# bwiberg/beam-radiance-estimate-pbrt

Measured on AMD Instinct MI355X. Metric: beam-radiance estimates/sec at 1M photons, higher is better.
Workload: dtype fp32

## Files before the change

### beam-radiance-estimate-pbrt_amd/csrc/bre_api_check.hip

```cpp
#include <cmath>
#include <cstring>
#include <vector>

#include "bre_ctx.h"

using namespace bre;

namespace {

bre_status check_hierarchy(bre_ctx *c, int64_t n, const float *x, int32_t n_aux, const float *aux, float *y) {
    if (n_aux < 2 || !aux) return fail(c, BRE_ERR_INVALID_ARG, "bre_device_check: kind 10 needs aux = (key_lo, leaf_size)");
    const int key_lo = (int)aux[0], K = (int)aux[1];
    if (n < 8 || n % 8 || !x || !y || key_lo < 0 || key_lo > 63 || K < 1 || K > 64 || n / 8 > ((int64_t)1 << 24))
        return fail(c, BRE_ERR_INVALID_ARG, "bre_device_check: kind 10 needs m <= 2^24 keys and boxes (8 words each), "
                    "key_lo in 0..63 and leaf_size in 1..64");
    const int64_t m = n / 8;
    std::vector<unsigned long long> keys((size_t)m);
    std::memcpy(keys.data(), x, (size_t)m * 8);
    for (int64_t i = 1; i < m; ++i)
        if ((keys[(size_t)i] >> key_lo) < (keys[(size_t)i - 1] >> key_lo))
            return fail(c, BRE_ERR_INVALID_ARG, "bre_device_check: kind 10 keys >> %d decrease at %lld: the hierarchy "
                        "kernels need a non-decreasing sequence", key_lo, (long long)i);
    std::vector<BeamRec> recs((size_t)m);
    const float *bx = x + 2 * m;
// ... 55 lines not shown
    int32_t head[8] = {0, 0, K, c->built_key_lo, (int32_t)nn, has4 ? 1 : 0, (int32_t)nleaf, 0};
    std::memcpy(head, &nv, sizeof(int64_t));
    std::memcpy(y, head, sizeof(head));
    if (nv == 0) return BRE_OK;
    BRE_TRY(set_device(c));
    float *keys = y + 8, *idx = keys + 2 * nv, *box = idx + nv, *nodes = box + 6 * nv, *lp = nodes + 16 * nn,
          *nodes4 = lp + nleaf;
    std::vector<BeamRec> recs((size_t)nv);
    HIPCHK(c, hipMemcpyAsync(keys, c->sort.keys_alt.ptr, (size_t)nv * 8, hipMemcpyDeviceToHost, c->stream));
    HIPCHK(c, hipMemcpyAsync(idx, c->sort.vals_alt.ptr, (size_t)nv * 4, hipMemcpyDeviceToHost, c->stream));
    HIPCHK(c, hipMemcpyAsync(recs.data(), c->recs.ptr, (size_t)nv * sizeof(BeamRec), hipMemcpyDeviceToHost, c->stream));
    HIPCHK(c, hipMemcpyAsync(nodes, c->nodes.ptr, (size_t)nn * sizeof(Node), hipMemcpyDeviceToHost, c->stream));
    if (nleaf > 1)
        HIPCHK(c, hipMemcpyAsync(lp, c->leaf_parent.ptr, (size_t)nleaf * 4, hipMemcpyDeviceToHost, c->stream));
    if (has4)
        HIPCHK(c, hipMemcpyAsync(nodes4, c->nodes4.ptr, (size_t)nn * sizeof(Node4), hipMemcpyDeviceToHost, c->stream));
    HIPCHK(c, hipStreamSynchronize(c->stream));
    if (nleaf == 1) std::memset(lp, 0, 4);
    for (int64_t i = 0; i < nv; ++i)
        for (int k = 0; k < 3; ++k) {
            box[6 * i + k] = recs[(size_t)i].lo[k];
            box[6 * i + 3 + k] = recs[(size_t)i].hi[k];
        }
    return BRE_OK;
}

}

extern "C" {

bre_status bre_device_check(bre_ctx *c, int32_t kind, int64_t n, const float *x, int32_t n_aux, const float *aux,
                            float *y) {
    if (!c) return BRE_ERR_INVALID_ARG;
    if (kind < 0 || kind > 14) return fail(c, BRE_ERR_INVALID_ARG, "bre_device_check: kind %d not in [0, 14]", kind);
    if (kind == 10) return check_hierarchy(c, n, x, n_aux, aux, y);
    if (kind == 11) return check_read_tree(c, n, y);
    if (n < 0 || (n > 0 && (!x || !y))) return fail(c, BRE_ERR_INVALID_ARG, "bre_device_check: bad arrays");
    if (kind == 12) {
        if (n % 6) return fail(c, BRE_ERR_INVALID_ARG, "bre_device_check: kind 12 needs whole records of 6 floats");
        if (n == 0) return BRE_OK;
        BRE_TRY(set_device(c));
        float *dx = nullptr, *dy = nullptr;
        HIPCHK(c, c->chk_x.get((size_t)n, &dx));
        HIPCHK(c, c->chk_y.get((size_t)n, &dy));
        HIPCHK(c, hipMemcpyAsync(dx, x, (size_t)n * 4, hipMemcpyHostToDevice, c->stream));
        HIPCHK(c, launch_check_specular(n / 6, dx, dy, c->stream));
        HIPCHK(c, hipMemcpyAsync(y, dy, (size_t)n * 4, hipMemcpyDeviceToHost, c->stream));
        HIPCHK(c, hipStreamSynchronize(c->stream));
        return BRE_OK;
    }
    if (kind == 13) {
        constexpr int kWords = (int)(sizeof(bre_material_ex) / 4);
        if (n % 9 || n_aux < kWords || n_aux % kWords || !aux)
            return fail(c, BRE_ERR_INVALID_ARG, "bre_device_check: kind 13 needs whole records of 9 floats and, in aux, "
                        "whole bre_material_ex records of %d words", kWords);
        const int n_mats = n_aux / kWords;
        std::vector<bre_material_ex> mats((size_t)n_mats);
        std::memcpy(mats.data(), aux, (size_t)n_aux * 4);
        std::vector<DevBsdf> table((size_t)n_mats);
        for (int k = 0; k < n_mats; ++k) {
            const std::string what = check_glossy_material(mats[(size_t)k]);
            if (!what.empty())
                return fail(c, BRE_ERR_INVALID_ARG, "bre_device_check: kind 13: material %d has %s", k, what.c_str());
            table[(size_t)k] = make_bsdf(mats[(size_t)k]);
        }
        for (int64_t i = 0; i < n / 9; ++i)
            if (!(x[9 * i + 8] >= 0 && x[9 * i + 8] < (float)n_mats) || x[9 * i + 8] != std::floor(x[9 * i + 8]))
                return fail(c, BRE_ERR_INVALID_ARG, "bre_device_check: kind 13: record %lld names material %g of %d",
                            (long long)i, (double)x[9 * i + 8], n_mats);
        if (n == 0) return BRE_OK;
// ... 167 lines not shown
```

### beam-radiance-estimate-pbrt_amd/csrc/bre_api_gather.hip

```cpp
#include <algorithm>

#include "bre_ctx.h"

using namespace bre;

namespace {

bre_status read_counters(bre_ctx *c, DevCounters *ctr) {
    if (!(c->timing || c->counters)) return BRE_OK;
    DevCounters h;
    HIPCHK(c, hipMemcpyAsync(&h, ctr, sizeof(h), hipMemcpyDeviceToHost, c->stream));
    HIPCHK(c, hipStreamSynchronize(c->stream));
    if (c->timing) {
        float ms = 0.f;
        HIPCHK(c, hipEventElapsedTime(&ms, c->ev[2], c->ev[3]));
        c->stats.gather_ms = ms;
    }
    c->stats.candidates = (int64_t)h.candidates;
    c->stats.contributions = (int64_t)h.contributions;
    c->stats.node_visits = (int64_t)h.node_visits;
    c->stats.leaf_visits = (int64_t)h.leaf_visits;
    c->stats.beam_evals = (int64_t)h.beam_evals;
    c->stats.ccp_wave_evals = (int64_t)h.ccp_wave_evals;
    c->stats.prefilter_rejects = (int64_t)h.prefilter_rejects;
// ... 121 lines not shown
    a.prefilter = c->prefilter;
    a.occupancy = c->occupancy;
    a.block_map = c->block_map;
    a.tscan = c->tscan >= 0 ? c->tscan : tscan_for(R + c->bset.radius);
    a.margin = c->margin;
    a.stack_cap = c->stack_cap;
    a.tile_spec = c->tile_spec;
    a.tile_budget = c->tile_budget;
    c->stats.tile_variant = 0;
    a.tile_variant = &c->stats.tile_variant;
    c->stats.n_segments = nseg;
    if (c->nvalid == 0) {
        HIPCHK(c, launch_zero_outputs(a, c->stream));
        return BRE_OK;
    }
    const int kernel = c->kernel;
    if (c->shard_mode == 2 && c->shard_count > 1 && (kernel == 2 || kernel == 5))
        return fail(c, BRE_ERR_STATE, "work-root shards (BRE_OPT_SHARD_MODE 2) need the tile kernel (BRE_OPT_KERNEL 0 or 4)");
    if (kernel == 5) {
        if (seg_index) return fail(c, BRE_ERR_STATE, "kernel 5 gathers in the caller's order only");
        return gather_chunk(c, a);
    }
    if (kernel == 2 && seg_index) return fail(c, BRE_ERR_STATE, "kernel 2 gathers in the caller's order only");
    if (kernel == 2) {
        if (c->timing) HIPCHK(c, hipEventRecord(c->ev[2], c->stream));
        HIPCHK(c, launch_gather_thread(a, c->counters, c->stream));
        if (c->timing) HIPCHK(c, hipEventRecord(c->ev[3], c->stream));
        return read_counters(c, a.ctr);
    }
    const bool want_cnt = c->counters || out.seg_counts;
    const bool rshard = c->shard_mode == 2 && c->shard_count > 1;
    const int S_eff = rshard ? (c->split + c->shard_count - 1) / c->shard_count : c->split;
    const size_t per_seg = (size_t)S_eff * (12 + (want_cnt ? 8 : 0));
    int64_t chunk = c->partial_cap / (int64_t)per_seg / 64 * 64;
    if (chunk > ((int64_t)1 << 26)) chunk = (int64_t)1 << 26;
    if (chunk < 64) chunk = 64;
    if (chunk > nseg) chunk = nseg;
    int32_t *roots = nullptr;
    HIPCHK(c, c->roots.get(kMaxSplit + 1, &roots));
    HIPCHK(c, c->partial.get(3 * (size_t)chunk * (size_t)S_eff, &a.partial));
    if (c->roots_split != c->split) {
        HIPCHK(c, c->roots_tmp.ensure(roots_scratch_bytes()));
        HIPCHK(c, launch_roots(a.nodes, c->split, roots, c->roots_tmp.ptr, c->stream));
        c->roots_split = c->split;
    }
    if (!c->nodes4_ok) {
        Node4 *nodes4 = nullptr;
        HIPCHK(c, c->nodes4.get((size_t)c->nnodes, &nodes4));
        HIPCHK(c, launch_collapse4(a.nodes, c->nnodes, nodes4, c->stream));
        c->nodes4_ok = true;
    }
    a.nodes4 = c->nodes4.as<Node4>();
    a.roots = roots;
    if (rshard) {
        int32_t *roots_sh = nullptr;
        HIPCHK(c, c->roots_sh.get(kMaxSplit + 1, &roots_sh));
        HIPCHK(c, launch_roots_shard(roots, c->split, c->shard_rank, c->shard_count, S_eff, roots_sh, c->stream));
        a.roots = roots_sh;
        a.split = S_eff;
    }
    HIPCHK(c, c->segrec.get((size_t)((chunk + 63) / 64 * 64), &a.segrec));
    if (want_cnt) HIPCHK(c, c->pcnt.get(2 * (size_t)chunk * (size_t)S_eff, &a.pcnt));
    if (c->tile_axis && a.leaf_size > 0) {
        const int64_t ntiles = (c->nvalid + a.leaf_size - 1) / a.leaf_size;
        HIPCHK(c, c->tileax.get((size_t)ntiles, &a.tileax));
        HIPCHK(c, c->segbox.get(8, &a.segbox));
    }
    if (c->timing) HIPCHK(c, hipEventRecord(c->ev[2], c->stream));
    if (!c->tile_ev) HIPCHK(c, hipEventCreateWithFlags(&c->tile_ev.h, hipEventDisableTiming));
    for (int64_t off = 0; off < nseg; off += chunk) {
        GatherArgs ac = a;
        ac.wait_ev = (off == 0 && c->after && c->after->tile_ev_valid) ? c->after->tile_ev.h : nullptr;
        ac.done_ev = off + chunk >= nseg ? c->tile_ev.h : nullptr;
        ac.user_start = off == 0 ? c->user_ev[0] : nullptr;
        ac.user_end = off + chunk >= nseg ? c->user_ev[1] : nullptr;
        ac.nseg = std::min(chunk, nseg - off);
        ac.seg = seg.slice(off);
        if (seg_index)
            ac.seg_index = seg_index + off;
        else
            ac.out = out.slice(off);
        HIPCHK(c, launch_gather_tile(ac, c->counters, c->stream));
    }
    c->tile_ev_valid = true;
    if (c->timing) HIPCHK(c, hipEventRecord(c->ev[3], c->stream));
    return read_counters(c, a.ctr);
}

bre_status gather_segments_core(bre_ctx *c, int64_t n, const SegView &seg, float R, int64_t npix,
                                const GatherOut &out) {
    const bool pshard = c->shard_mode == 1 && c->shard_count > 1;
    const bool sortable = c->kernel == 0 || c->kernel == 4;
    const bool seg_out = out.seg_rgb || out.seg_counts;
    if (n < 0 || npix < 0) return fail(c, BRE_ERR_INVALID_ARG, "bre_gather: negative size");
    if (n > 0 && (!seg.o || !seg.p || !seg.d || !seg.t))
        return fail(c, BRE_ERR_INVALID_ARG, "bre_gather: null segment array");
    if (out.accum && !seg.pix) return fail(c, BRE_ERR_INVALID_ARG, "bre_gather: accum_rgb given without seg_pixel");
    if (pshard && seg_out) {
        if (!sortable) return fail(c, BRE_ERR_STATE, "packet shards with per-segment outputs need kernel 0 or 4");
        GatherArgs z{};
        z.nseg = n;
        z.out = out;
        HIPCHK(c, launch_zero_outputs(z, c->stream));
    }
    const auto pick = [&](const SegView &from, const int32_t *index) -> bre_status {
        const int64_t m = bre_shard_segments(n, c->shard_rank, c->shard_count, c->shard_block);
        c->stats.n_segments = m;
        if (m == 0) return BRE_OK;
        SegArrays &sp = c->sp;
        int32_t *sp_index = nullptr;
        HIPCHK(c, sp.ensure((size_t)m));
        if (seg_out) HIPCHK(c, c->sp_index.get((size_t)m, &sp_index));
        const PacketPick pk{n, m, c->shard_rank, c->shard_count, c->shard_block, from, index, sp.out(), sp_index};
        HIPCHK(c, launch_packet_pick(pk, c->stream));
        SegView picked = sp.view();
// ... 185 lines not shown
```

### beam-radiance-estimate-pbrt_amd/csrc/bre_ctx.h

```cpp
#pragma once
#include <hip/hip_runtime.h>

#include <cstddef>
#include <cstdint>
#include <cstring>
#include <initializer_list>
#include <string>
#include <vector>

#include "../../include/bre.h"
#include "bre_device.h"
#include "bre_trace.h"

#ifndef BRE_KERNEL_READBACK
#define BRE_KERNEL_READBACK 1
#endif
#ifndef BRE_TILE_BUDGET
#define BRE_TILE_BUDGET 7
#endif
static_assert(BRE_TILE_BUDGET == 6 || BRE_TILE_BUDGET == 7, "BRE_TILE_BUDGET must be 6 or 7");

namespace bre {

struct NoCopy {
// ... 143 lines not shown
};

struct SceneDevice {
    DevMem tris, nodes, prims, light_tri, light_func, light_cdf, dlights, mats, bsdfs, lobes, lobes_mx;
    DevScene head;
    uint64_t hash = 0;
    std::vector<unsigned char> bytes[4];
    DevMem md_table, md_pairs, md_light, md_dens;
    bool media_stale = false;
    DevMem grid;
    std::vector<unsigned char> grid_bytes;
    DevMem record;
    std::vector<unsigned char> record_bytes;
};

}

struct bre_ctx {
    int device = 0;
    bre::Stream stream;
    bre::Stream pstream;
    bre::Event ev[4];
    bre::Event fork_ev, join_ev;
    bre::Event tile_ev;
    bool tile_ev_valid = false;
    hipEvent_t user_ev[2] = {nullptr, nullptr};
    bre::PinnedWords flags_host;
    bre::PinnedWords rb_host;
    std::string err;
    bool counters = false, timing = false, prefilter = true, sort_segments = true;
    int kernel = 0, leaf_size = 1, sqrt_mode = 0, split = 256, leaf2 = 64, chunk_len = 400, chunk_leaf = 1;
    int shard_rank = 0, shard_count = 1, shard_block = 1, shard_mode = 0, film_classes = 1;
    int stack_cap = 0, occupancy = 6, sort_key = 4, block_map = 3, tscan = -1;
    int64_t partial_cap = (int64_t)4 << 30;
    int beam_key = 2, margin = 1, tile_axis = 1, split_records = 0, film_compose = 1;
    int photon_single = 1, pass_priority = 1, kernel_readback = BRE_KERNEL_READBACK;
    int slot_passes = 1, coarse_keys = 0, stage_all = 0, tile_spec = 1;
    int tile_budget = BRE_TILE_BUDGET;
    int64_t nbeams = 0, nvalid = 0, nnodes = 0;
    bre::BeamSet bset;
    int built_leaf_size = 1;
    int built_key_lo = 0;
    bool build_scratch_ok = false;
    int roots_split = -1;
    bool nodes4_ok = false;
    bool beams_kept = false;
    bre::BeamArrays in;
    bre::DevMem box, cent, cbounds, nvalid_buf, leaf_parent, visit, gbox;
    bre::SortScratch sort;
    bre::DevMem recs, pow, nodes;
    bre::SegArrays g;
    bre::DevMem g_accum, g_seg_rgb, g_counts;
    bre::DevMem counters_buf, roots, roots_sh, roots_tmp, partial, pcnt, segrec, tileax, segbox, nodes4;
    bre::DevMem ch_bounds, ch_counts, ch_offsets, ch_range, ch_scan_tmp, ch_box, ch_cent, ch_slo, ch_shi, ch_par,
        ch_recs, ch_cpar, ch_nodes;
    int64_t n_chunks = 0;
    bre::DevMem ss_bounds;
    bre::SortScratch ss_sort;
    bre::SegArrays ss;
    bre::SegArrays sp;
    bre::DevMem sp_index;
    bre::DevMem px_seg, px_cls;
    bre::SortScratch px_sort;
    bre::SceneState held;
    bre::SceneDevice dev;
    int seg_budget = 16;
    bre::DevMem ph_counts, ph_offsets, ph_tmp;
    bre::BeamArrays ph_s;
    bre::DevMem cam_dev, cam_perms, cam_offs, cam_tmp, cam_flags;
    bre::SegArrays cs;
    bre::DevMem cs_valid;
    bre::SegArrays seg;
    bre::DevMem seg_depth;
    int64_t cam_nseg = 0;
    int64_t cam_npix = 0;
    int cam_w = -1, cam_h = -1;
    bre_scene cam_scene;
    bre::DevMem chk_x, chk_aux, chk_y;
    int lds_per_block = 0;
    bre_stats stats;
    bre_ctx *after = nullptr;
    std::vector<bre_ctx *> followers;
};

namespace bre {

// ... 81 lines not shown
```

### beam-radiance-estimate-pbrt_amd/csrc/bre_device.h

```cpp
#pragma once

#include <hip/hip_runtime.h>
#include <stdint.h>

#include "bre_views.h"

namespace bre {

struct alignas(16) BeamRec {
    float lo[3], hi[3];
    float b0[3];
    float bu[3];
    float mag_b;
    float radius;
    float pad[2];
};
struct BeamSet {
    int uniform = 0;
    float radius = 0.f;
};
__device__ __forceinline__ float beam_radius(const BeamSet &u, float rec_radius) {
    return u.uniform ? u.radius : rec_radius;
}
static_assert(sizeof(BeamRec) == 64, "BeamRec must be one 64-B line");

struct alignas(16) Node {
    float lo[2][3];
    float hi[2][3];
    int32_t child[2];
    int32_t parent;
    int32_t nleaf;
};
static_assert(sizeof(Node) == 64, "Node must be one 64-B line");

constexpr int32_t kEmptyChild = INT32_MIN;

struct alignas(16) Node4 {
// ... 77 lines not shown
    float invs[3];
    float inv_mag_a;
};
static_assert(sizeof(SegRec) == 64, "SegRec must be one 64-B line");
__device__ __forceinline__ const float4 *seg_plane(const SegRec *base, int64_t s, int k) {
    return reinterpret_cast<const float4 *>(base) + ((s >> 6) << 8) + (k << 6) + (s & 63);
}

struct alignas(16) TileAxis {
    float d[3], thr;
    float m[3], grow;
};

struct GatherArgs {
    int64_t nseg;
    SegView seg;
    float R;
    int64_t npix;
    GatherOut out;
    const int32_t *seg_index;
    const BeamRec *recs;
    const float4 *pow;
    BeamSet bset;
    const Node *nodes;
    const Node4 *nodes4 = nullptr;
    int64_t nvalid;
    int leaf_size;
    DevCounters *ctr;
    const int32_t *roots;
    int split;
    float *partial;
    int32_t *pcnt;
    SegRec *segrec;
    bool prefilter;
    int occupancy;
    int stack_cap;
    int block_map;
    int tscan;
    int margin;
    int tile_spec = 1;
    int tile_budget = 7;
    int64_t *tile_variant = nullptr;
    TileAxis *tileax;
    unsigned int *segbox;
    hipEvent_t wait_ev = nullptr;
    hipEvent_t done_ev = nullptr;
    hipEvent_t user_start = nullptr, user_end = nullptr;
};

struct ChunkBuild {
    const BeamRec *parents;
    BeamSet bset;
    int64_t nparents;
    const float *seg_o, *seg_p;
    int64_t nseg;
    float R;
    float len_factor;
    unsigned int *seg_bounds;
    unsigned int *cbounds;
    int32_t *counts;
    int64_t *offsets;
    float *range;
    void *scan_tmp;
    size_t scan_tmp_bytes;
};
size_t chunk_scan_temp_bytes(int64_t n);
// ... 44 lines not shown
    const uint8_t *cls;
    int classes;
    unsigned int *keys, *keys_alt;
    int32_t *vals, *vals_alt;
    void *tmp;
    size_t tmp_bytes;
    unsigned int *flags;
    unsigned int bad_pixel_flag;
    int slot = 1;
};
size_t pixel_sort_temp_bytes(int64_t n);
hipError_t launch_pixel_compose(const PixelCompose &c, hipStream_t st);
hipError_t launch_seg_classes(int64_t n, int block, int classes, const int32_t *perm, uint8_t *cls, hipStream_t st);
hipError_t launch_film_add(int64_t m, float *src, float *dst, int clear, hipStream_t st);
hipError_t launch_resolve_classes(int64_t m, int classes, const float *in, float *out, hipStream_t st);
constexpr int kFilmSources = 8;
struct FilmSources {
    const float *src[kFilmSources];
    int n;
};
hipError_t launch_film_sum(const FilmSources &t, int64_t m, float *dst, int accumulate, hipStream_t st);

hipError_t launch_sort_segments(const SegSort &s, hipStream_t st);
struct PacketPick {
    int64_t n, m;
    int rank, count, chunk;
    SegView in;
    const int32_t *index;
    SegOut out;
    int32_t *index2;
};
hipError_t launch_packet_pick(const PacketPick &k, hipStream_t st);

hipError_t launch_device_check(int kind, int64_t n, const float *x, int n_aux, const float *aux, float *y,
                               hipStream_t s);

hipError_t slot_fill(void *p, int64_t nwords, unsigned int value, hipStream_t s);
size_t slot_scan_temp_bytes(int64_t n);
hipError_t slot_exclusive_scan(const int32_t *in, int64_t *out, int64_t n, int64_t *total, void *tmp, hipStream_t s);
size_t slot_sort_temp_bytes(int64_t n, int key_bytes);
hipError_t slot_sort_pairs(void *tmp, const unsigned long long *k0, unsigned long long *k1, const int32_t *v0,
                           int32_t *v1, int64_t n, int begin_bit, int end_bit, hipStream_t s);
hipError_t slot_sort_pairs(void *tmp, const unsigned int *k0, unsigned int *k1, const int32_t *v0, int32_t *v1,
                           int64_t n, int begin_bit, int end_bit, hipStream_t s);

size_t roots_scratch_bytes();
hipError_t launch_roots(const Node *nodes, int S, int32_t *roots, void *scratch, hipStream_t s);
hipError_t launch_collapse4(const Node *nodes, int64_t nnodes, Node4 *out, hipStream_t s);
hipError_t launch_roots_shard(const int32_t *roots, int S, int rank, int count, int S2, int32_t *out,
                              hipStream_t s);
hipError_t launch_gather_thread(const GatherArgs &a, bool counters, hipStream_t s);
hipError_t launch_tile_axis(const GatherArgs &a, hipStream_t s);
hipError_t launch_gather_tile(const GatherArgs &a, bool counters, hipStream_t s);
hipError_t launch_zero_outputs(const GatherArgs &a, hipStream_t s);

}
```

### beam-radiance-estimate-pbrt_amd/csrc/bre_gather.hip

```cpp
#include <hip/hip_runtime.h>

#include <float.h>

#include "bre_device.h"
#include "bre_lane.h"
#include "bre_math.h"

namespace bre {

namespace {

#ifndef BRE_PHASE_TIMING
#define BRE_PHASE_TIMING 0
#endif
#ifndef BRE_SQRT_NOSCALE
#define BRE_SQRT_NOSCALE 1
#endif
__device__ __forceinline__ __amdgpu_buffer_rsrc_t buf_rsrc(const void *p) {
    return __builtin_amdgcn_make_buffer_rsrc(const_cast<void *>(p), (short)0, -1, 0x00020000);
}
__device__ __forceinline__ float4 buf_f4(__amdgpu_buffer_rsrc_t r, unsigned int voff, unsigned int soff) {
    const auto v = __builtin_amdgcn_raw_buffer_load_b128(r, (int)voff, (int)soff, 0);
    return make_float4(__int_as_float(v[0]), __int_as_float(v[1]), __int_as_float(v[2]), __int_as_float(v[3]));
}
// ... 314 lines not shown
            a.x += v.x;
            a.y += v.y;
            a.z += v.z;
            a.w += v.w;
            sh.acc[sl] = a;
        }
    };
#pragma unroll
    for (int k = 0; k < 8; ++k) {
        if (__ballot(rank == k) == 0ull) return;
        round_k(k);
    }
#pragma nounroll
    for (int k = 8; k < 64; ++k) {
        if (__ballot(rank == k) == 0ull) return;
        round_k(k);
    }
}

template <bool FIXED_>
struct TileCfg {
    static constexpr bool kFixed = FIXED_;
    static constexpr int kPrefilter = 1, kMargin = 1, kMap = 3, kLeaf = 64;
};
using TileGeneric = TileCfg<false>;
using TileProd = TileCfg<true>;
template <bool COUNT, int MINW, class CFG = TileGeneric>
__global__ __launch_bounds__(kTileBlock, MINW) void k_gather_tile(
    int64_t nseg, const float *__restrict__ so, const float *__restrict__ sp_, const float *__restrict__ sd,
    const float *__restrict__ stmax, const SegRec *__restrict__ srec, float R, float *__restrict__ partial,
    int32_t *__restrict__ pcnt_arg, const BeamRec *__restrict__ recs, const float4 *__restrict__ pw, BeamSet bset_arg,
    const Node *__restrict__ nodes, const Node4 *__restrict__ nodes4, int64_t nvalid, int leaf_size_arg,
    const int32_t *__restrict__ roots, int S, DevCounters *ctr, int stack_cap, int prefilter_arg, int map_arg, int tscan,
    int margin_arg, const TileAxis *__restrict__ tax) {
    constexpr bool FIXED = CFG::kFixed;
    static_assert(!(FIXED && COUNT), "the counting instantiation is generic");
    const int prefilter = FIXED ? CFG::kPrefilter : prefilter_arg;
    const int map = FIXED ? CFG::kMap : map_arg;
    const int margin = FIXED ? CFG::kMargin : margin_arg;
    const int leaf_size = FIXED ? CFG::kLeaf : leaf_size_arg;
    int32_t *const pcnt = FIXED ? nullptr : pcnt_arg;
    const BeamSet bset{FIXED ? 1 : bset_arg.uniform, bset_arg.radius};
    __shared__ TileSharedT<FIXED> shm[kTileBlock / 64];
    int sub;
    int64_t grp;
    if (map == 3) {
        const unsigned P = gridDim.x / (unsigned)S;
        grp = blockIdx.x % P;
        sub = (int)(blockIdx.x / P);
    } else if (map == 1) {
        grp = blockIdx.x / (unsigned)S;
        sub = (int)((blockIdx.x % (unsigned)S + grp) % (unsigned)S);
    } else if (map == 2 || S < 8) {
        sub = (int)(blockIdx.x % (unsigned)S);
        grp = blockIdx.x / (unsigned)S;
    } else {
        const unsigned per = (unsigned)S >> 3;
        const unsigned q = blockIdx.x >> 3;
        sub = (int)((blockIdx.x & 7u) * per + q % per);
        grp = q / per;
    }
    if (sub >= roots[S]) return;
    const int w = threadIdx.x >> 6, lane = threadIdx.x & 63;
    wave_time(0, lane);
    TileSharedT<FIXED> &sh = shm[w];
    const int64_t s = grp * kTileBlock + threadIdx.x;
    const int64_t seg0 = grp * kTileBlock + (int64_t)__builtin_amdgcn_readfirstlane(w) * 64;
    const bool count_c = COUNT || pcnt != nullptr;
    Lane L;
    bool valid;
    if constexpr (FIXED) {
        zero_lane(L);
        valid = s < nseg;
        if (valid) {
            const float4 *q = seg_plane(srec, s, 0);
            const float4 a0 = q[0], a1 = q[64], a2 = q[128];
            L.o = mk(a0.x, a0.y, a0.z);
            L.tmax = a0.w;
            L.p = mk(a1.x, a1.y, a1.z);
            L.mag_a = fabsf(a1.w);
            L.au = mk(a2.x, a2.y, a2.z);
            L.d = mk(sd[3 * s], sd[3 * s + 1], sd[3 * s + 2]);
            L.omax = fmaxf(fmaxf(fabsf(L.o.x), fabsf(L.o.y)), fabsf(L.o.z)) + L.mag_a;
        }
    } else {
        valid = load_lane(s, nseg, so, sp_, sd, stmax, L);
    }
    Bundle K;
    K.delta = FLT_MAX;
    K.gbox = FLT_MAX;
    if (prefilter && __ballot(valid) != 0ull) K = make_bundle(L, valid);
    const ScanLane SL = make_scan_lane(L, margin);
    const float al_max = uniform_f(wave_max(valid && SL.al < FLT_MAX ? SL.al : 0.f));
    const float inv_maxd = bset.uniform ? uniform_f(1.0f / (R + bset.radius)) : 0.f;
    sh.acc[lane] = make_float4(0.f, 0.f, 0.f, 0.f);
    __builtin_amdgcn_wave_barrier();
    int cand = 0;
    unsigned long long visits = 0;
    Prof pf;
    int t1 = 0;
    int64_t cur_first = 0;
    unsigned long long ph_stage = 0, ph_scan = 0, ph_exact = 0;
    unsigned long long ss_on = 0, ss_kept = 0, ss_steps = 0, ss_pairs = 0, ss_leaves = 0, ss_q = 0, ss_min = 0,
                       ss_tr = 0;
    const unsigned long long ph_t0 = phase_clock();

    const int discard = TileSharedT<FIXED>::kDiscard + lane;
    const auto push = [&](unsigned long long m, int32_t e_beam, int32_t e_lane) {
        if (m == 0ull) return;
        int rank = (int)__builtin_amdgcn_mbcnt_hi((unsigned)(m >> 32),
                                                  __builtin_amdgcn_mbcnt_lo((unsigned)m, (unsigned)t1));
        if constexpr (FIXED) {
            if (__builtin_amdgcn_inverse_ballot_w64(m)) sh.q[rank].e = QEntry{e_beam, e_lane};
        } else {
            asm volatile("" : "+v"(rank));
            const int slot = __builtin_amdgcn_inverse_ballot_w64(m) ? rank : discard;
            sh.q[slot].e = QEntry{e_beam, e_lane};
        }
        t1 += __popcll(m);
        if (COUNT) pf.queued += __popcll(m);
        if (BRE_SCAN_STATS) ss_q += __popcll(m);
    };
    const auto drain = [&]() {
        if (t1 < 64) return;
        __builtin_amdgcn_wave_barrier();
        const unsigned long long d0 = BRE_PHASE_TIMING ? phase_clock() : 0ull;
        int h = 0;
// ... 262 lines not shown
        atomicAdd(&ctr->node_visits, ph_exact);
        atomicAdd(&ctr->leaf_visits, phase_clock() - ph_t0);
    }
    if (COUNT) {
        unsigned long long rj = pf.rejects;
#pragma unroll
        for (int off = 32; off >= 1; off >>= 1) rj += __shfl_xor(rj, off);
        if (lane == 0) {
            atomicAdd(&ctr->node_visits, visits);
            atomicAdd(&ctr->leaf_visits, pf.leaves);
            atomicAdd(&ctr->beam_evals, pf.beams);
            atomicAdd(&ctr->useful_beam_evals, pf.useful);
            atomicAdd(&ctr->prefilter_rejects, rj);
            atomicAdd(&ctr->ccp_wave_evals, pf.ccp_waves);
            atomicAdd(&ctr->queued_pairs, pf.queued);
        }
    }
}

__global__ __launch_bounds__(kPassBlock) void k_seg_prep(int64_t nseg, const float *__restrict__ so,
                                                  const float *__restrict__ sp_, const float *__restrict__ sd,
                                                  const float *__restrict__ stmax, SegRec *__restrict__ out) {
    const int64_t s = (int64_t)blockIdx.x * kPassBlock + threadIdx.x;
    if (s >= nseg) return;
    Lane L;
    load_lane(s, nseg, so, sp_, sd, stmax, L);
    float4 *q = const_cast<float4 *>(seg_plane(out, s, 0));
    q[0] = make_float4(L.o.x, L.o.y, L.o.z, L.tmax);
    q[64] = make_float4(L.p.x, L.p.y, L.p.z, L.has_inf ? -L.mag_a : L.mag_a);
    q[128] = make_float4(L.au.x, L.au.y, L.au.z, __int_as_float(L.has_inf ? 1 : 0));
    q[192] = make_float4(L.invs.x, L.invs.y, L.invs.z, L.mag_a != 0.0f ? 1.0f / L.mag_a : 0.0f);
}

__global__ __launch_bounds__(kPassBlock) void k_reduce(int64_t nseg, const float *__restrict__ partial,
                                                const int32_t *__restrict__ pcnt, const int32_t *__restrict__ roots,
                                                int S, const int32_t *__restrict__ pixel, int64_t npix,
                                                float *__restrict__ accum, float *__restrict__ seg_rgb,
                                                int32_t *__restrict__ seg_counts, const int32_t *__restrict__ seg_index,
                                                DevCounters *ctr) {
    const int64_t s = (int64_t)blockIdx.x * kPassBlock + threadIdx.x;
    const bool in = s < nseg;
    const int nr = roots[S];
    float cr = 0.f, cg = 0.f, cb = 0.f;
    long long c = 0, k = 0;
    if (in) {
        for (int j = 0; j < nr; ++j) {
            const float *q = partial + 3 * ((int64_t)j * nseg + s);
            cr += q[0];
            cg += q[1];
            cb += q[2];
            if (pcnt) {
                c += pcnt[2 * ((int64_t)j * nseg + s)];
                k += pcnt[2 * ((int64_t)j * nseg + s) + 1];
            }
        }
        const int64_t so = seg_index ? (int64_t)seg_index[s] : s;
        if (seg_rgb) {
            seg_rgb[3 * so] = cr;
            seg_rgb[3 * so + 1] = cg;
            seg_rgb[3 * so + 2] = cb;
        }
        if (seg_counts) {
            seg_counts[2 * so] = c < 0 ? -1 : (int32_t)c;
            seg_counts[2 * so + 1] = (int32_t)k;
        }
        if (accum) {
// ... 15 lines not shown
            uk += __shfl_xor(uk, off);
        }
        if ((threadIdx.x & 63) == 0) {
            atomicAdd(&ctr->candidates, uc);
            atomicAdd(&ctr->contributions, uk);
        }
    }
}

__global__ void k_zero_seg(int64_t nseg, float *__restrict__ seg_rgb, int32_t *__restrict__ seg_counts,
                           const int32_t *__restrict__ seg_index) {
    const int64_t i = (int64_t)blockIdx.x * 64 + threadIdx.x;
    if (i >= nseg) return;
    const int64_t s = seg_index ? (int64_t)seg_index[i] : i;
    if (seg_rgb) {
        seg_rgb[3 * s] = 0.f;
        seg_rgb[3 * s + 1] = 0.f;
        seg_rgb[3 * s + 2] = 0.f;
    }
    if (seg_counts) {
        seg_counts[2 * s] = 0;
        seg_counts[2 * s + 1] = 0;
    }
}

}

hipError_t launch_gather_tile(const GatherArgs &a, bool counters, hipStream_t s) {
    if (a.nseg == 0) return hipSuccess;
    const int stack_cap = a.stack_cap > 0 ? a.stack_cap : kStackDepth;
    if (stack_cap > kStackDepth) return hipErrorInvalidValue;
    int32_t *pcnt = (counters || a.out.seg_counts) ? a.pcnt : nullptr;
    if ((counters || a.out.seg_counts) && !pcnt) return hipErrorInvalidValue;
    if (!a.segrec || a.leaf_size > 64) return hipErrorInvalidValue;
    if (!a.nodes4) return hipErrorInvalidValue;
    hipLaunchKernelGGL(k_seg_prep, dim3((unsigned int)((a.nseg + kPassBlock - 1) / kPassBlock)), dim3(kPassBlock), 0, s, a.nseg, a.seg.o, a.seg.p, a.seg.d,
                       a.seg.t, a.segrec);
    const TileAxis *tax = nullptr;
    if (a.tileax && a.segbox && a.prefilter && a.nvalid > 0) {
        const hipError_t ea = launch_tile_axis(a, s);
        if (ea != hipSuccess) return ea;
        tax = a.tileax;
    }
    const dim3 grid4((unsigned int)(((a.nseg + kTileBlock - 1) / kTileBlock) * a.split));
    const int block_map = (a.block_map == 0 && (a.split & 7) != 0) ? 3 : a.block_map;
    if (a.wait_ev) {
        const hipError_t ew = hipStreamWaitEvent(s, a.wait_ev, 0);
        if (ew != hipSuccess) return ew;
    }
    if (a.user_start) {
        const hipError_t es = hipEventRecord(a.user_start, s);
        if (es != hipSuccess) return es;
    }
    const bool fixed = a.tile_spec && !counters && pcnt == nullptr && a.occupancy == 6 && a.prefilter &&
                       a.margin == TileProd::kMargin && block_map == TileProd::kMap &&
                       a.leaf_size == TileProd::kLeaf && tax != nullptr && a.bset.uniform != 0;
    if (a.tile_variant) *a.tile_variant = fixed ? 2 : 1;
#define BRE_LAUNCH_TILE(C, W, CFG)                                                                               \
    hipLaunchKernelGGL((k_gather_tile<C, W, CFG>), grid4, dim3(kTileBlock), 0, s, a.nseg, a.seg.o, a.seg.p,      \
                       a.seg.d, a.seg.t, a.segrec, a.R, a.partial, pcnt, a.recs, a.pow, a.bset, a.nodes,         \
                       a.nodes4, a.nvalid, a.leaf_size, a.roots, a.split, a.ctr, stack_cap, (int)a.prefilter,    \
                       block_map, a.tscan, a.margin, tax)
    if (counters) {
        BRE_LAUNCH_TILE(true, 1, TileGeneric);
    } else if (fixed && a.tile_budget == 7) {
        BRE_LAUNCH_TILE(false, 7, TileProd);
    } else if (fixed) {
        BRE_LAUNCH_TILE(false, 6, TileProd);
    } else if (a.occupancy == 1) {
        BRE_LAUNCH_TILE(false, 1, TileGeneric);
    } else if (a.occupancy == 4) {
        BRE_LAUNCH_TILE(false, 4, TileGeneric);
    } else if (a.occupancy == 5) {
        BRE_LAUNCH_TILE(false, 5, TileGeneric);
    } else if (a.occupancy == 6) {
        BRE_LAUNCH_TILE(false, 6, TileGeneric);
    } else if (a.occupancy == 8) {
        BRE_LAUNCH_TILE(false, 8, TileGeneric);
    } else {
        BRE_LAUNCH_TILE(false, 7, TileGeneric);
    }
#undef BRE_LAUNCH_TILE
    hipError_t e4 = hipGetLastError();
    if (e4 != hipSuccess) return e4;
    if (a.done_ev) {
        e4 = hipEventRecord(a.done_ev, s);
        if (e4 != hipSuccess) return e4;
    }
    if (a.user_end) {
        e4 = hipEventRecord(a.user_end, s);
        if (e4 != hipSuccess) return e4;
    }
    hipLaunchKernelGGL(k_reduce, dim3((unsigned int)((a.nseg + kPassBlock - 1) / kPassBlock)), dim3(kPassBlock), 0, s, a.nseg, a.partial, pcnt,
                       a.roots, a.split, a.seg.pix, a.npix, a.out.accum, a.out.seg_rgb, a.out.seg_counts, a.seg_index, a.ctr);
    return hipGetLastError();
}

hipError_t launch_zero_outputs(const GatherArgs &a, hipStream_t s) {
    if (a.nseg == 0 || (!a.out.seg_rgb && !a.out.seg_counts)) return hipSuccess;
    hipLaunchKernelGGL(k_zero_seg, dim3((unsigned int)((a.nseg + 63) / 64)), dim3(64), 0, s, a.nseg, a.out.seg_rgb,
                       a.out.seg_counts, a.seg_index);
    return hipGetLastError();
}

}

#if BRE_WAVE_TIMES
extern "C" int bre_study_wave_times(int64_t n, unsigned long long *out) {
    if (n > bre::kWaveTimes) n = bre::kWaveTimes;
    if (hipDeviceSynchronize() != hipSuccess) return 2;
    if (hipMemcpyFromSymbol(out, HIP_SYMBOL(bre::g_wave_t), (size_t)n * 8, 0, hipMemcpyDeviceToHost) != hipSuccess) return 2;
    if (hipMemcpyFromSymbol(out + n, HIP_SYMBOL(bre::g_wave_t), (size_t)n * 8, (size_t)bre::kWaveTimes * 8,
                            hipMemcpyDeviceToHost) != hipSuccess)
        return 2;
    return 0;
}
#endif
```

Baseline: 4.454 million.

## Precompute per-packet bundle and scan bounds in a prep kernel for tile gather

Adds a k_packet_prep kernel that computes each 64-segment packet's bundle (cone, box, scan parameters, al_max) once and stores it in a PacketRec buffer. The fixed-config (TileProd, budget 7) tile kernel then loads this record instead of rebuilding the bundle, skipping the wave reductions and some segment loads. The aim is to stop repeating this per-packet setup in every one of the split blocks that share a packet. In exchange it adds an extra kernel launch and buffer per chunk, and a new device check (kind 15) to validate the precomputed records.

```diff
diff --git a/beam-radiance-estimate-pbrt_amd/csrc/bre_api_check.hip b/beam-radiance-estimate-pbrt_amd/csrc/bre_api_check.hip
--- a/beam-radiance-estimate-pbrt_amd/csrc/bre_api_check.hip
+++ b/beam-radiance-estimate-pbrt_amd/csrc/bre_api_check.hip
@@ -111,10 +111,42 @@
 bre_status bre_device_check(bre_ctx *c, int32_t kind, int64_t n, const float *x, int32_t n_aux, const float *aux,
                             float *y) {
     if (!c) return BRE_ERR_INVALID_ARG;
-    if (kind < 0 || kind > 14) return fail(c, BRE_ERR_INVALID_ARG, "bre_device_check: kind %d not in [0, 14]", kind);
+    if (kind < 0 || kind > 15) return fail(c, BRE_ERR_INVALID_ARG, "bre_device_check: kind %d not in [0, 15]", kind);
     if (kind == 10) return check_hierarchy(c, n, x, n_aux, aux, y);
     if (kind == 11) return check_read_tree(c, n, y);
     if (n < 0 || (n > 0 && (!x || !y))) return fail(c, BRE_ERR_INVALID_ARG, "bre_device_check: bad arrays");
+    if (kind == 15) {
+        if (n % 10 || n == 0) return fail(c, BRE_ERR_INVALID_ARG, "bre_device_check: kind 15 needs whole segments of 10 floats");
+        const int64_t ns = n / 10;
+        if (c->pktrec_nseg != ns || !c->pktrec.ptr)
+            return fail(c, BRE_ERR_STATE, "bre_device_check: kind 15: the context's last tile launch gathered %lld "
+                        "segments, not %lld", (long long)c->pktrec_nseg, (long long)ns);
+        BRE_TRY(set_device(c));
+        std::vector<float> soa((size_t)n);
+        float *ho = soa.data(), *hp = ho + 3 * ns, *hd = hp + 3 * ns, *ht = hd + 3 * ns;
+        for (int64_t i = 0; i < ns; ++i) {
+            for (int k = 0; k < 3; ++k) {
+                ho[3 * i + k] = x[10 * i + k];
+                hp[3 * i + k] = x[10 * i + 3 + k];
+                hd[3 * i + k] = x[10 * i + 6 + k];
+            }
+            ht[i] = x[10 * i + 9];
+        }
+        float *dx = nullptr;
+        unsigned int *dy = nullptr;
+        HIPCHK(c, c->chk_x.get((size_t)n, &dx));
+        HIPCHK(c, c->chk_y.get((size_t)1, &dy));
+        HIPCHK(c, hipMemcpyAsync(dx, soa.data(), (size_t)n * 4, hipMemcpyHostToDevice, c->stream));
+        HIPCHK(c, hipMemsetAsync(dy, 0, 4, c->stream));
+        const SegView sv{dx, dx + 3 * ns, dx + 6 * ns, dx + 9 * ns, nullptr};
+        HIPCHK(c, launch_packet_check(ns, sv, c->pktrec.as<PacketRec>(), dy, c->stream));
+        unsigned int bad = 0;
+        HIPCHK(c, hipMemcpyAsync(&bad, dy, 4, hipMemcpyDeviceToHost, c->stream));
+        HIPCHK(c, hipStreamSynchronize(c->stream));
+        y[0] = (float)bad;
+        y[1] = (float)packet_count(ns);
+        return BRE_OK;
+    }
     if (kind == 12) {
         if (n % 6) return fail(c, BRE_ERR_INVALID_ARG, "bre_device_check: kind 12 needs whole records of 6 floats");
         if (n == 0) return BRE_OK;
diff --git a/beam-radiance-estimate-pbrt_amd/csrc/bre_api_gather.hip b/beam-radiance-estimate-pbrt_amd/csrc/bre_api_gather.hip
--- a/beam-radiance-estimate-pbrt_amd/csrc/bre_api_gather.hip
+++ b/beam-radiance-estimate-pbrt_amd/csrc/bre_api_gather.hip
@@ -177,10 +177,7 @@
     const bool rshard = c->shard_mode == 2 && c->shard_count > 1;
     const int S_eff = rshard ? (c->split + c->shard_count - 1) / c->shard_count : c->split;
     const size_t per_seg = (size_t)S_eff * (12 + (want_cnt ? 8 : 0));
-    int64_t chunk = c->partial_cap / (int64_t)per_seg / 64 * 64;
-    if (chunk > ((int64_t)1 << 26)) chunk = (int64_t)1 << 26;
-    if (chunk < 64) chunk = 64;
-    if (chunk > nseg) chunk = nseg;
+    const int64_t chunk = launch_chunk(nseg, c->partial_cap, per_seg);
     int32_t *roots = nullptr;
     HIPCHK(c, c->roots.get(kMaxSplit + 1, &roots));
     HIPCHK(c, c->partial.get(3 * (size_t)chunk * (size_t)S_eff, &a.partial));
@@ -205,6 +202,7 @@
         a.split = S_eff;
     }
     HIPCHK(c, c->segrec.get((size_t)((chunk + 63) / 64 * 64), &a.segrec));
+    HIPCHK(c, c->pktrec.get((size_t)packet_count(chunk), &a.pktrec));
     if (want_cnt) HIPCHK(c, c->pcnt.get(2 * (size_t)chunk * (size_t)S_eff, &a.pcnt));
     if (c->tile_axis && a.leaf_size > 0) {
         const int64_t ntiles = (c->nvalid + a.leaf_size - 1) / a.leaf_size;
@@ -226,6 +224,7 @@
         else
             ac.out = out.slice(off);
         HIPCHK(c, launch_gather_tile(ac, c->counters, c->stream));
+        c->pktrec_nseg = ac.nseg;
     }
     c->tile_ev_valid = true;
     if (c->timing) HIPCHK(c, hipEventRecord(c->ev[3], c->stream));
diff --git a/beam-radiance-estimate-pbrt_amd/csrc/bre_ctx.h b/beam-radiance-estimate-pbrt_amd/csrc/bre_ctx.h
--- a/beam-radiance-estimate-pbrt_amd/csrc/bre_ctx.h
+++ b/beam-radiance-estimate-pbrt_amd/csrc/bre_ctx.h
@@ -199,6 +199,7 @@
     int kernel = 0, leaf_size = 1, sqrt_mode = 0, split = 256, leaf2 = 64, chunk_len = 400, chunk_leaf = 1;
     int shard_rank = 0, shard_count = 1, shard_block = 1, shard_mode = 0, film_classes = 1;
     int stack_cap = 0, occupancy = 6, sort_key = 4, block_map = 3, tscan = -1;
+    int64_t pktrec_nseg = 0;
     int64_t partial_cap = (int64_t)4 << 30;
     int beam_key = 2, margin = 1, tile_axis = 1, split_records = 0, film_compose = 1;
     int photon_single = 1, pass_priority = 1, kernel_readback = BRE_KERNEL_READBACK;
@@ -218,7 +219,7 @@
     bre::DevMem recs, pow, nodes;
     bre::SegArrays g;
     bre::DevMem g_accum, g_seg_rgb, g_counts;
-    bre::DevMem counters_buf, roots, roots_sh, roots_tmp, partial, pcnt, segrec, tileax, segbox, nodes4;
+    bre::DevMem counters_buf, roots, roots_sh, roots_tmp, partial, pcnt, segrec, pktrec, tileax, segbox, nodes4;
     bre::DevMem ch_bounds, ch_counts, ch_offsets, ch_range, ch_scan_tmp, ch_box, ch_cent, ch_slo, ch_shi, ch_par,
         ch_recs, ch_cpar, ch_nodes;
     int64_t n_chunks = 0;
diff --git a/beam-radiance-estimate-pbrt_amd/csrc/bre_device.h b/beam-radiance-estimate-pbrt_amd/csrc/bre_device.h
--- a/beam-radiance-estimate-pbrt_amd/csrc/bre_device.h
+++ b/beam-radiance-estimate-pbrt_amd/csrc/bre_device.h
@@ -3,6 +3,7 @@
 #include <hip/hip_runtime.h>
 #include <stdint.h>
 
+#include "bre_packet.h"
 #include "bre_views.h"
 
 namespace bre {
@@ -146,6 +147,7 @@
     float *partial;
     int32_t *pcnt;
     SegRec *segrec;
+    PacketRec *pktrec = nullptr;
     bool prefilter;
     int occupancy;
     int stack_cap;
@@ -256,6 +258,8 @@
 };
 hipError_t launch_packet_pick(const PacketPick &k, hipStream_t st);
 
+hipError_t launch_packet_check(int64_t nseg, const SegView &seg, const PacketRec *pktrec, unsigned int *bad,
+                               hipStream_t s);
 hipError_t launch_device_check(int kind, int64_t n, const float *x, int n_aux, const float *aux, float *y,
                                hipStream_t s);
 
diff --git a/beam-radiance-estimate-pbrt_amd/csrc/bre_gather.hip b/beam-radiance-estimate-pbrt_amd/csrc/bre_gather.hip
--- a/beam-radiance-estimate-pbrt_amd/csrc/bre_gather.hip
+++ b/beam-radiance-estimate-pbrt_amd/csrc/bre_gather.hip
@@ -370,8 +370,9 @@
     int32_t *__restrict__ pcnt_arg, const BeamRec *__restrict__ recs, const float4 *__restrict__ pw, BeamSet bset_arg,
     const Node *__restrict__ nodes, const Node4 *__restrict__ nodes4, int64_t nvalid, int leaf_size_arg,
     const int32_t *__restrict__ roots, int S, DevCounters *ctr, int stack_cap, int prefilter_arg, int map_arg, int tscan,
-    int margin_arg, const TileAxis *__restrict__ tax) {
+    int margin_arg, const TileAxis *__restrict__ tax, const PacketRec *__restrict__ pkr, float inv_maxd_arg) {
     constexpr bool FIXED = CFG::kFixed;
+    constexpr bool PREP = FIXED && MINW == 7;
     static_assert(!(FIXED && COUNT), "the counting instantiation is generic");
     const int prefilter = FIXED ? CFG::kPrefilter : prefilter_arg;
     const int map = FIXED ? CFG::kMap : map_arg;
@@ -412,14 +413,17 @@
         valid = s < nseg;
         if (valid) {
             const float4 *q = seg_plane(srec, s, 0);
-            const float4 a0 = q[0], a1 = q[64], a2 = q[128];
+            const float4 a0 = q[0], a2 = q[128];
             L.o = mk(a0.x, a0.y, a0.z);
             L.tmax = a0.w;
-            L.p = mk(a1.x, a1.y, a1.z);
-            L.mag_a = fabsf(a1.w);
             L.au = mk(a2.x, a2.y, a2.z);
-            L.d = mk(sd[3 * s], sd[3 * s + 1], sd[3 * s + 2]);
-            L.omax = fmaxf(fmaxf(fabsf(L.o.x), fabsf(L.o.y)), fabsf(L.o.z)) + L.mag_a;
+            if constexpr (!PREP) {
+                const float4 a1 = q[64];
+                L.p = mk(a1.x, a1.y, a1.z);
+                L.mag_a = fabsf(a1.w);
+                L.d = mk(sd[3 * s], sd[3 * s + 1], sd[3 * s + 2]);
+                L.omax = fmaxf(fmaxf(fabsf(L.o.x), fabsf(L.o.y)), fabsf(L.o.z)) + L.mag_a;
+            }
         }
     } else {
         valid = load_lane(s, nseg, so, sp_, sd, stmax, L);
@@ -427,10 +431,30 @@
     Bundle K;
     K.delta = FLT_MAX;
     K.gbox = FLT_MAX;
-    if (prefilter && __ballot(valid) != 0ull) K = make_bundle(L, valid);
-    const ScanLane SL = make_scan_lane(L, margin);
-    const float al_max = uniform_f(wave_max(valid && SL.al < FLT_MAX ? SL.al : 0.f));
-    const float inv_maxd = bset.uniform ? uniform_f(1.0f / (R + bset.radius)) : 0.f;
+    float al_max, inv_maxd;
+    ScanLane SL;
+    if constexpr (PREP) {
+        const PacketRec &P = pkr[packet_index(seg0)];
+        K.co = mk(P.co[0], P.co[1], P.co[2]);
+        K.cu = mk(P.cu[0], P.cu[1], P.cu[2]);
+        K.delta = P.delta;
+        K.omax = P.omax;
+        K.s0 = P.s0;
+        K.s1 = P.s1;
+        K.gbox = P.gbox;
+        K.icu = mk(P.icu[0], P.icu[1], P.icu[2]);
+        K.q = mk(P.q[0], P.q[1], P.q[2]);
+        K.col1 = P.col1;
+        al_max = P.al_max;
+        inv_maxd = inv_maxd_arg;
+        SL.q = make_scan_lane(L, margin).q;
+        SL.al = 0.f;
+    } else {
+        if (prefilter && __ballot(valid) != 0ull) K = make_bundle(L, valid);
+        SL = make_scan_lane(L, margin);
+        al_max = uniform_f(wave_max(valid && SL.al < FLT_MAX ? SL.al : 0.f));
+        inv_maxd = bset.uniform ? uniform_f(1.0f / (R + bset.radius)) : 0.f;
+    }
     sh.acc[lane] = make_float4(0.f, 0.f, 0.f, 0.f);
     __builtin_amdgcn_wave_barrier();
     int cand = 0;
@@ -759,6 +783,64 @@
     q[192] = make_float4(L.invs.x, L.invs.y, L.invs.z, L.mag_a != 0.0f ? 1.0f / L.mag_a : 0.0f);
 }
 
+__device__ __forceinline__ PacketRec make_packet_rec(int64_t s, int64_t nseg, const float *__restrict__ so,
+                                                     const float *__restrict__ sp_, const float *__restrict__ sd,
+                                                     const float *__restrict__ stmax) {
+    Lane L;
+    const bool valid = load_lane(s, nseg, so, sp_, sd, stmax, L);
+    Bundle K;
+    K.delta = FLT_MAX;
+    K.gbox = FLT_MAX;
+    K.co = K.cu = K.icu = K.q = mk(0.f, 0.f, 0.f);
+    K.omax = K.s0 = K.s1 = K.col1 = 0.f;
+    if (__ballot(valid) != 0ull) K = make_bundle(L, valid);
+    const ScanLane SL = make_scan_lane(L, TileProd::kMargin);
+    PacketRec P;
+    P.co[0] = K.co.x, P.co[1] = K.co.y, P.co[2] = K.co.z;
+    P.cu[0] = K.cu.x, P.cu[1] = K.cu.y, P.cu[2] = K.cu.z;
+    P.delta = K.delta;
+    P.omax = K.omax;
+    P.s0 = K.s0;
+    P.s1 = K.s1;
+    P.gbox = K.gbox;
+    P.icu[0] = K.icu.x, P.icu[1] = K.icu.y, P.icu[2] = K.icu.z;
+    P.q[0] = K.q.x, P.q[1] = K.q.y, P.q[2] = K.q.z;
+    P.col1 = K.col1;
+    P.al_max = uniform_f(wave_max(valid && SL.al < FLT_MAX ? SL.al : 0.f));
+    P.pad = 0.f;
+    return P;
+}
+
+__global__ __launch_bounds__(64, 7) void k_packet_prep(int64_t nseg, const float *__restrict__ so,
+                                                       const float *__restrict__ sp_, const float *__restrict__ sd,
+                                                       const float *__restrict__ stmax, PacketRec *__restrict__ out) {
+    const int64_t s = (int64_t)blockIdx.x * 64 + threadIdx.x;
+    const PacketRec P = make_packet_rec(s, nseg, so, sp_, sd, stmax);
+    const float *w = reinterpret_cast<const float *>(&P);
+    float v = 0.f;
+#pragma unroll
+    for (int k = 0; k < kPacketRecWords; ++k) v = (int)threadIdx.x == k ? w[k] : v;
+    if ((int)threadIdx.x < kPacketRecWords)
+        reinterpret_cast<float *>(out + blockIdx.x)[threadIdx.x] = v;
+}
+
+__global__ __launch_bounds__(64) void k_packet_check(int64_t nseg, const float *__restrict__ so,
+                                                     const float *__restrict__ sp_, const float *__restrict__ sd,
+                                                     const float *__restrict__ stmax,
+                                                     const PacketRec *__restrict__ in, unsigned int *__restrict__ bad) {
+    const int64_t s = (int64_t)blockIdx.x * 64 + threadIdx.x;
+    const PacketRec P = make_packet_rec(s, nseg, so, sp_, sd, stmax);
+    const unsigned int *w = reinterpret_cast<const unsigned int *>(&P);
+    unsigned int v = 0u;
+#pragma unroll
+    for (int k = 0; k < kPacketRecWords; ++k) v = (int)threadIdx.x == k ? w[k] : v;
+    bool differs = false;
+    if ((int)threadIdx.x < kPacketRecWords)
+        differs = reinterpret_cast<const unsigned int *>(in + blockIdx.x)[threadIdx.x] != v;
+    const int n = __popcll(__ballot(differs));
+    if (threadIdx.x == 0 && n != 0) atomicAdd(bad, (unsigned int)n);
+}
+
 __global__ __launch_bounds__(kPassBlock) void k_reduce(int64_t nseg, const float *__restrict__ partial,
                                                 const int32_t *__restrict__ pcnt, const int32_t *__restrict__ roots,
                                                 int S, const int32_t *__restrict__ pixel, int64_t npix,
@@ -840,10 +922,12 @@
     if (stack_cap > kStackDepth) return hipErrorInvalidValue;
     int32_t *pcnt = (counters || a.out.seg_counts) ? a.pcnt : nullptr;
     if ((counters || a.out.seg_counts) && !pcnt) return hipErrorInvalidValue;
-    if (!a.segrec || a.leaf_size > 64) return hipErrorInvalidValue;
+    if (!a.segrec || !a.pktrec || a.leaf_size > 64) return hipErrorInvalidValue;
     if (!a.nodes4) return hipErrorInvalidValue;
     hipLaunchKernelGGL(k_seg_prep, dim3((unsigned int)((a.nseg + kPassBlock - 1) / kPassBlock)), dim3(kPassBlock), 0, s, a.nseg, a.seg.o, a.seg.p, a.seg.d,
                        a.seg.t, a.segrec);
+    hipLaunchKernelGGL(k_packet_prep, dim3((unsigned int)packet_count(a.nseg)), dim3(64), 0, s, a.nseg, a.seg.o, a.seg.p,
+                       a.seg.d, a.seg.t, a.pktrec);
     const TileAxis *tax = nullptr;
     if (a.tileax && a.segbox && a.prefilter && a.nvalid > 0) {
         const hipError_t ea = launch_tile_axis(a, s);
@@ -864,11 +948,13 @@
                        a.margin == TileProd::kMargin && block_map == TileProd::kMap &&
                        a.leaf_size == TileProd::kLeaf && tax != nullptr && a.bset.uniform != 0;
     if (a.tile_variant) *a.tile_variant = fixed ? 2 : 1;
+    const float maxd = a.R + a.bset.radius;
+    const float inv_maxd = a.bset.uniform ? 1.0f / maxd : 0.f;
 #define BRE_LAUNCH_TILE(C, W, CFG)                                                                               \
     hipLaunchKernelGGL((k_gather_tile<C, W, CFG>), grid4, dim3(kTileBlock), 0, s, a.nseg, a.seg.o, a.seg.p,      \
                        a.seg.d, a.seg.t, a.segrec, a.R, a.partial, pcnt, a.recs, a.pow, a.bset, a.nodes,         \
                        a.nodes4, a.nvalid, a.leaf_size, a.roots, a.split, a.ctr, stack_cap, (int)a.prefilter,    \
-                       block_map, a.tscan, a.margin, tax)
+                       block_map, a.tscan, a.margin, tax, a.pktrec, inv_maxd)
     if (counters) {
         BRE_LAUNCH_TILE(true, 1, TileGeneric);
     } else if (fixed && a.tile_budget == 7) {
@@ -904,6 +990,14 @@
     return hipGetLastError();
 }
 
+hipError_t launch_packet_check(int64_t nseg, const SegView &seg, const PacketRec *pktrec, unsigned int *bad,
+                               hipStream_t s) {
+    if (nseg <= 0) return hipSuccess;
+    hipLaunchKernelGGL(k_packet_check, dim3((unsigned int)packet_count(nseg)), dim3(64), 0, s, nseg, seg.o, seg.p, seg.d,
+                       seg.t, pktrec, bad);
+    return hipGetLastError();
+}
+
 hipError_t launch_zero_outputs(const GatherArgs &a, hipStream_t s) {
     if (a.nseg == 0 || (!a.out.seg_rgb && !a.out.seg_counts)) return hipSuccess;
     hipLaunchKernelGGL(k_zero_seg, dim3((unsigned int)((a.nseg + 63) / 64)), dim3(64), 0, s, a.nseg, a.out.seg_rgb,
diff --git a/beam-radiance-estimate-pbrt_amd/csrc/bre_packet.h b/beam-radiance-estimate-pbrt_amd/csrc/bre_packet.h
--- /dev/null
+++ b/beam-radiance-estimate-pbrt_amd/csrc/bre_packet.h
@@ -0,0 +1,32 @@
+#pragma once
+
+#include <stddef.h>
+#include <stdint.h>
+
+namespace bre {
+
+struct alignas(16) PacketRec {
+    float co[3], cu[3];
+    float delta, omax;
+    float s0, s1, gbox;
+    float icu[3];
+    float q[3];
+    float col1;
+    float al_max;
+    float pad;
+};
+static_assert(sizeof(PacketRec) == 80 && sizeof(PacketRec) % 16 == 0, "PacketRec must be a multiple of 16 B");
+constexpr int kPacketRecWords = (int)(sizeof(PacketRec) / sizeof(float));
+
+constexpr int64_t packet_count(int64_t nseg) { return nseg <= 0 ? 0 : (nseg + 63) / 64; }
+constexpr int64_t packet_index(int64_t seg0) { return seg0 >> 6; }
+
+inline int64_t launch_chunk(int64_t nseg, int64_t partial_cap, size_t per_seg) {
+    int64_t chunk = partial_cap / (int64_t)per_seg / 64 * 64;
+    if (chunk > ((int64_t)1 << 26)) chunk = (int64_t)1 << 26;
+    if (chunk < 64) chunk = 64;
+    if (chunk > nseg) chunk = nseg;
+    return chunk;
+}
+
+}
```

New measurement: 4.521 million (median of 6 runs). 1.5% higher.
